# a-r-r-o-w/finetrainers

Measured on NVIDIA H100. Metric: latent_tokens_per_sec, higher is better.
Workload: dtype bf16

## Files before the change

### finetrainers_b200/csrc/b2d_attn.cu

```cuda
#include <float.h>
#include <stdlib.h>
#include <type_traits>
#include "b2d_internal.h"
#include "b2d_ptx.cuh"

namespace b2d {

constexpr int ATT_THREADS = 384;
constexpr int TILE = 128;
constexpr int PANEL = 64;
constexpr int TILE_PANEL_BYTES = TILE * PANEL * 2;
constexpr int HALF_PANEL_BYTES = 64 * PANEL * 2;
constexpr int ATT_SMEM_LIMIT = 227 * 1024;
constexpr float LOG2E = 1.4426950408889634f;
constexpr float LN2 = 0.6931471805599453f;

template <int HD>
struct AttnShape {
    static_assert(HD == 64 || HD == 128, "attention is built for head_dim 64 and 128");
    static constexpr int PANELS = HD / PANEL;
    static constexpr int TILE_BYTES = PANELS * TILE_PANEL_BYTES;
};

__device__ __forceinline__ float fast_exp2(float x) {
    float y;
    asm("ex2.approx.ftz.f32 %0, %1;" : "=f"(y) : "f"(x));
    return y;
}

template <int KK>
__device__ __forceinline__ void acc_to_a(const float (&s)[8 * KK], uint32_t (&a)[KK][4]) {
#pragma unroll
    for (int kk = 0; kk < KK; ++kk) {
        a[kk][0] = pack_bf16x2(s[8 * kk + 0], s[8 * kk + 1]);
        a[kk][1] = pack_bf16x2(s[8 * kk + 2], s[8 * kk + 3]);
        a[kk][2] = pack_bf16x2(s[8 * kk + 4], s[8 * kk + 5]);
        a[kk][3] = pack_bf16x2(s[8 * kk + 6], s[8 * kk + 7]);
    }
}

template <int N, int HD, int XP, int YP>
__device__ __forceinline__ void mma_xyt(float (&s)[N / 2], uint32_t x_smem, uint32_t y_smem) {
    const uint32_t xlo = sdesc_lo_kmajor(x_smem), ylo = sdesc_lo_kmajor(y_smem);
#pragma unroll
    for (int k = 0; k < HD / 16; ++k) {
        const uint32_t xk = xlo + (k / 4) * (XP >> 4) + (k % 4) * SDESC_KSTEP_KMAJOR;
        const uint32_t yk = ylo + (k / 4) * (YP >> 4) + (k % 4) * SDESC_KSTEP_KMAJOR;
        Wgmma<N, 0, 0>::ss(s, sdesc(xk), sdesc(yk), k > 0 ? 1u : 0u);
    }
}

template <int KK, int HD, int ZP>
__device__ __forceinline__ void mma_az(float (&o)[HD / 2], const uint32_t (&a)[KK][4], uint32_t z_smem) {
    const uint32_t zlo = HD == PANEL ? sdesc_lo_mnmajor(z_smem) : sdesc_lo_mnmajor(z_smem, ZP);
#pragma unroll
    for (int kk = 0; kk < KK; ++kk) Wgmma<HD, 0, 1>::rs(o, a[kk], sdesc(zlo + kk * SDESC_KSTEP_MNMAJOR), 1u);
}

template <int HD, int P>
__device__ __forceinline__ void tma_load_tile(uint8_t* dst, const CUtensorMap* m, uint64_t* bar, int h, int row, int b) {
#pragma unroll
    for (int i = 0; i < HD / PANEL; ++i) tma_load_4d(dst + i * P, m, bar, i * PANEL, h, row, b);
}

struct AttnFwdParams {
    CUtensorMap tmQ, tmK, tmV;
    const float* key_bias;
    __nv_bfloat16* out;
    float* lse;
    int B, H, Sq, Sk;
    float scale_log2;
};

template <int HD>
constexpr int FWD_STAGES = HD == 64 ? 3 : 2;
template <int HD>
constexpr int FWD_SMEM = AttnShape<HD>::TILE_BYTES  + FWD_STAGES<HD> * 2 * AttnShape<HD>::TILE_BYTES  + 1024 + 256;
static_assert(FWD_SMEM<64> <= ATT_SMEM_LIMIT && FWD_SMEM<128> <= ATT_SMEM_LIMIT, "attn_fwd shared memory");

template <int HD>
__global__ void __launch_bounds__(ATT_THREADS, 1) attn_fwd_kernel(const __grid_constant__ AttnFwdParams p) {
    constexpr int TILE_BYTES = AttnShape<HD>::TILE_BYTES, STAGES = FWD_STAGES<HD>;
    griddep_launch_dependents();
    extern __shared__ uint8_t smem_raw[];
    uint8_t* smem = reinterpret_cast<uint8_t*>((reinterpret_cast<uintptr_t>(smem_raw) + 1023) & ~uintptr_t(1023));
    uint8_t* sQ = smem;
    uint8_t* sKV = smem + TILE_BYTES;
    uint64_t* q_bar = reinterpret_cast<uint64_t*>(sKV + STAGES * 2 * TILE_BYTES);
    uint64_t* full_bar = q_bar + 1;
    uint64_t* empty_bar = full_bar + STAGES;

    const int warp = threadIdx.x >> 5, lane = threadIdx.x & 31;
    const int qt = blockIdx.x, bh = blockIdx.y;
    const int b = bh / p.H, h = bh % p.H;
    const int n_kt = (p.Sk + TILE - 1) / TILE;

    if (threadIdx.x == 0) {
        tma_prefetch_desc(&p.tmQ);
        tma_prefetch_desc(&p.tmK);
        tma_prefetch_desc(&p.tmV);
        mbar_init(q_bar, 1);
        for (int i = 0; i < STAGES; ++i) {
            mbar_init(&full_bar[i], 1);
            mbar_init(&empty_bar[i], 256);
        }
        fence_mbar_init();
    }
    __syncthreads();
    griddep_wait();

    if (warp < 4) {
        setmaxnreg_dec<40>();
        if (warp == 0 && elect_one()) {
            mbar_expect_tx(q_bar, TILE_BYTES);
            tma_load_tile<HD, TILE_PANEL_BYTES>(sQ, &p.tmQ, q_bar, h, qt * TILE, b);
            int stage = 0;
            uint32_t phase = 0;
            for (int j = 0; j < n_kt; ++j) {
                mbar_wait(&empty_bar[stage], phase ^ 1);
                uint8_t* sK = sKV + stage * 2 * TILE_BYTES;
                mbar_expect_tx(&full_bar[stage], 2 * TILE_BYTES);
                tma_load_tile<HD, TILE_PANEL_BYTES>(sK, &p.tmK, &full_bar[stage], h, j * TILE, b);
                tma_load_tile<HD, TILE_PANEL_BYTES>(sK + TILE_BYTES, &p.tmV, &full_bar[stage], h, j * TILE, b);
                if (++stage == STAGES) {
                    stage = 0;
                    phase ^= 1;
                }
            }
        }
        return;
    }
    setmaxnreg_inc<232>();
    const int cw = (warp >> 2) - 1, wq = warp & 3;
    const int qd = lane & 3;
    const uint32_t q_smem = smem_u32(sQ) + cw * HALF_PANEL_BYTES;
    const float* kb = p.key_bias ? p.key_bias + (long long)b * p.Sk : nullptr;
    const float sl2 = p.scale_log2;

    float kbias[32];
    auto bias_of = [&](int key) { return (kb != nullptr && key < p.Sk) ? kb[key] * LOG2E : 0.f; };
    auto load_bias = [&](int j) {
        if (HD != 64) return;
#pragma unroll
        for (int jj = 0; jj < 16; ++jj)
#pragma unroll
            for (int e = 0; e < 2; ++e) {
                const int key = j * TILE + 8 * jj + 2 * qd + e;
                kbias[2 * jj + e] = bias_of(key);
            }
    };
    float o[HD / 2];
#pragma unroll
    for (int i = 0; i < HD / 2; ++i) o[i] = 0.f;
    float m[2] = {-FLT_MAX, -FLT_MAX}, l[2] = {0.f, 0.f};
    auto softmax = [&](float (&s)[64], int j, float (&corr)[2]) {
        float mx[2] = {-INFINITY, -INFINITY};
        if ((j + 1) * TILE > p.Sk) {
#pragma unroll
            for (int jj = 0; jj < 16; ++jj)
#pragma unroll
                for (int e = 0; e < 2; ++e) {
                    const int key = j * TILE + 8 * jj + 2 * qd + e;
                    const float bias = HD == 64 ? kbias[2 * jj + e] : bias_of(key);
#pragma unroll
                    for (int hh = 0; hh < 2; ++hh) {
                        float v = key < p.Sk ? fmaf(s[4 * jj + 2 * hh + e], sl2, bias) : -INFINITY;
                        s[4 * jj + 2 * hh + e] = v;
                        mx[hh] = fmaxf(mx[hh], v);
                    }
                }
        } else {
#pragma unroll
            for (int jj = 0; jj < 16; ++jj)
#pragma unroll
                for (int e = 0; e < 2; ++e) {
                    const float bias = HD == 64 ? kbias[2 * jj + e] : bias_of(j * TILE + 8 * jj + 2 * qd + e);
#pragma unroll
                    for (int hh = 0; hh < 2; ++hh) {
                        float v = fmaf(s[4 * jj + 2 * hh + e], sl2, bias);
                        s[4 * jj + 2 * hh + e] = v;
                        mx[hh] = fmaxf(mx[hh], v);
                    }
                }
        }
#pragma unroll
        for (int hh = 0; hh < 2; ++hh) {
            mx[hh] = fmaxf(mx[hh], __shfl_xor_sync(0xffffffffu, mx[hh], 1));
            mx[hh] = fmaxf(mx[hh], __shfl_xor_sync(0xffffffffu, mx[hh], 2));
            const float mn = fmaxf(m[hh], mx[hh]);
            corr[hh] = fast_exp2(m[hh] - mn);
            m[hh] = mn;
            l[hh] *= corr[hh];
        }
#pragma unroll
        for (int jj = 0; jj < 16; ++jj)
#pragma unroll
            for (int hh = 0; hh < 2; ++hh)
#pragma unroll
                for (int e = 0; e < 2; ++e) {
                    const float pv = fast_exp2(s[4 * jj + 2 * hh + e] - m[hh]);
                    s[4 * jj + 2 * hh + e] = pv;
                    l[hh] += pv;
                }
    };
    auto rescale_o = [&](const float (&corr)[2]) {
#pragma unroll
        for (int jj = 0; jj < HD / 8; ++jj)
#pragma unroll
            for (int hh = 0; hh < 2; ++hh) {
                o[4 * jj + 2 * hh] *= corr[hh];
                o[4 * jj + 2 * hh + 1] *= corr[hh];
            }
    };
    auto turn_begin = [&] { named_bar_sync(1 + cw, 256); };
    auto turn_end = [&](bool last) {
        if (cw == 0 || !last) named_bar_arrive(2 - cw, 256);
    };
    if (cw == 1) named_bar_arrive(1, 256);

    mbar_wait(q_bar, 0);
    float s[64], corr[2];
    uint32_t pa[8][4];
    int stage = 0;
    uint32_t phase = 0;
    mbar_wait(&full_bar[0], 0);
    turn_begin();
    wgmma_fence();
    mma_xyt<128, HD, TILE_PANEL_BYTES, TILE_PANEL_BYTES>(s, q_smem, smem_u32(sKV));
    wgmma_commit();
    turn_end(false);
    load_bias(0);
    wgmma_wait<0>();
    wgmma_fence_regs(s);
    softmax(s, 0, corr);
    acc_to_a<8>(s, pa);
    for (int j = 1; j < n_kt; ++j) {
        const int prev = stage;
        if (++stage == STAGES) {
            stage = 0;
            phase ^= 1;
        }
        mbar_wait(&full_bar[stage], phase);
        turn_begin();
        wgmma_fence();
        mma_xyt<128, HD, TILE_PANEL_BYTES, TILE_PANEL_BYTES>(s, q_smem, smem_u32(sKV + stage * 2 * TILE_BYTES));
        wgmma_commit();
        mma_az<8, HD, TILE_PANEL_BYTES>(o, pa, smem_u32(sKV + prev * 2 * TILE_BYTES) + TILE_BYTES);
        wgmma_commit();
        turn_end(false);
        load_bias(j);
        wgmma_wait<1>();
        wgmma_fence_regs(s);
        softmax(s, j, corr);
        wgmma_wait<0>();
        wgmma_fence_regs(o);
        mbar_arrive(&empty_bar[prev]);
        rescale_o(corr);
        acc_to_a<8>(s, pa);
    }
    turn_begin();
    wgmma_fence();
    mma_az<8, HD, TILE_PANEL_BYTES>(o, pa, smem_u32(sKV + stage * 2 * TILE_BYTES) + TILE_BYTES);
    wgmma_commit();
    turn_end(true);
    wgmma_wait<0>();
    wgmma_fence_regs(o);
    mbar_arrive(&empty_bar[stage]);
#pragma unroll
    for (int hh = 0; hh < 2; ++hh) {
        l[hh] += __shfl_xor_sync(0xffffffffu, l[hh], 1);
        l[hh] += __shfl_xor_sync(0xffffffffu, l[hh], 2);
    }
    const int r0 = qt * TILE + cw * 64 + wq * 16 + (lane >> 2);
#pragma unroll
    for (int hh = 0; hh < 2; ++hh) {
        const int row = r0 + 8 * hh;
        if (row >= p.Sq) continue;
        const bool any = l[hh] > 0.f;
        const float inv = any ? 1.f / l[hh] : 0.f;
        __nv_bfloat16* orow = p.out + (((long long)b * p.Sq + row) * p.H + h) * HD;
#pragma unroll
        for (int jj = 0; jj < HD / 8; ++jj)
            *reinterpret_cast<uint32_t*>(orow + 8 * jj + 2 * qd) =
                pack_bf16x2(o[4 * jj + 2 * hh] * inv, o[4 * jj + 2 * hh + 1] * inv);
        if (qd == 0) p.lse[(long long)bh * p.Sq + row] = any ? (m[hh] + __log2f(l[hh])) * LN2 : INFINITY;
    }
}

template <int HD>
__global__ void attn_delta_kernel(const __nv_bfloat16* __restrict__ out, const __nv_bfloat16* __restrict__ dout,
                                  const float* __restrict__ lse, float* __restrict__ delta, float* __restrict__ nlse2,
                                  int B, int H, int Sq) {
    constexpr int LANES = HD / 8, LOG2_LANES = HD == 64 ? 3 : 4;
    static_assert((1 << LOG2_LANES) == LANES, "lanes per head row");
    griddep_launch_dependents();
    griddep_wait();
    const long long t = (long long)blockIdx.x * blockDim.x + threadIdx.x;
    const long long total = (long long)B * Sq * H * LANES;
    const bool ok = t < total;
    const long long e0 = (ok ? t : 0) * 8;
    uint4 a = *reinterpret_cast<const uint4*>(out + e0);
    uint4 d = *reinterpret_cast<const uint4*>(dout + e0);
    float acc = bf16_lo(a.x) * bf16_lo(d.x) + bf16_hi(a.x) * bf16_hi(d.x) + bf16_lo(a.y) * bf16_lo(d.y) +
                bf16_hi(a.y) * bf16_hi(d.y) + bf16_lo(a.z) * bf16_lo(d.z) + bf16_hi(a.z) * bf16_hi(d.z) +
                bf16_lo(a.w) * bf16_lo(d.w) + bf16_hi(a.w) * bf16_hi(d.w);
#pragma unroll
    for (int o = 1; o < LANES; o <<= 1) acc += __shfl_xor_sync(0xffffffffu, acc, o);
    if (ok && (t & (LANES - 1)) == 0) {
        const long long hr = t >> LOG2_LANES;
        const int h = (int)(hr % H);
        const long long bq = hr / H;
        const int q = (int)(bq % Sq);
        const int b = (int)(bq / Sq);
        const long long o = ((long long)b * H + h) * Sq + q;
        delta[o] = acc;
        nlse2[o] = -lse[o] * LOG2E;
    }
}

struct AttnBwdParams {
    CUtensorMap tmX1, tmX2, tmY1, tmY2;
    const float* key_bias;
    const float* delta;
    const float* nlse2;
    __nv_bfloat16* out1;
    __nv_bfloat16* out2;
    float* acc1;
    float* acc2;
    long long part_stride;
    int y_per_split;
    int B, H, Sq, Sk;
    float scale, scale_log2;
};

constexpr int ATT_MAX_SPLITS = 8;
template <int HD, int YR>
struct BwdShape {
    static_assert(YR == 64 || YR == 128, "streamed tiles are 64 or 128 rows");
    static constexpr int Y_PANEL_BYTES = YR * PANEL * 2;
    static constexpr int Y_BYTES = AttnShape<HD>::PANELS * Y_PANEL_BYTES;
    static constexpr int COLS = 2 * YR;
    static constexpr int STAGES = HD == 64 && YR == 128 ? 3 : 4;
    static constexpr int SMEM = 2 * AttnShape<HD>::TILE_BYTES + STAGES * (2 * Y_BYTES + COLS * 4) + 1024 + 256;
};
static_assert(BwdShape<64, 64>::SMEM <= ATT_SMEM_LIMIT && BwdShape<64, 128>::SMEM <= ATT_SMEM_LIMIT &&
                  BwdShape<128, 64>::SMEM <= ATT_SMEM_LIMIT,
              "attn_bwd shared memory");
template <int HD>
constexpr int BWD_REGS_PRODUCER = HD == 64 ? 40 : 24;
template <int HD>
constexpr int BWD_REGS_MATH = HD == 64 ? 232 : 240;
static_assert(BWD_REGS_PRODUCER<64> * 128 + BWD_REGS_MATH<64> * 256 == 168 * ATT_THREADS &&
                  BWD_REGS_PRODUCER<128> * 128 + BWD_REGS_MATH<128> * 256 == 168 * ATT_THREADS,
              "setmaxnreg split");

template <bool DKV, int HD, int YR>
__global__ void __launch_bounds__(ATT_THREADS, 1) attn_bwd_kernel(const __grid_constant__ AttnBwdParams p) {
    using Shape = BwdShape<HD, YR>;
    constexpr int TILE_BYTES = AttnShape<HD>::TILE_BYTES, Y_BYTES = Shape::Y_BYTES, STAGES = Shape::STAGES;
    constexpr int COLS = Shape::COLS, KK = YR / 16;
    griddep_launch_dependents();
    extern __shared__ uint8_t smem_raw[];
    uint8_t* smem = reinterpret_cast<uint8_t*>((reinterpret_cast<uintptr_t>(smem_raw) + 1023) & ~uintptr_t(1023));
    uint8_t* sX = smem;
    uint8_t* sY = smem + 2 * TILE_BYTES;
    float* sC = reinterpret_cast<float*>(sY + STAGES * 2 * Y_BYTES);
    uint64_t* x_bar = reinterpret_cast<uint64_t*>(sC + STAGES * COLS);
    uint64_t* full_bar = x_bar + 1;
    uint64_t* empty_bar = full_bar + STAGES;

    const int warp = threadIdx.x >> 5, lane = threadIdx.x & 31;
    const int xt = blockIdx.x, bh = blockIdx.y;
    const int b = bh / p.H, h = bh % p.H;
    const int S_x = DKV ? p.Sk : p.Sq, S_y = DKV ? p.Sq : p.Sk;
    const int y_begin = blockIdx.z * p.y_per_split;
    auto y_end_of_slice = [&] { return min((S_y + YR - 1) / YR, y_begin + p.y_per_split); };

    if (threadIdx.x == 0) {
        tma_prefetch_desc(&p.tmX1);
        tma_prefetch_desc(&p.tmX2);
        tma_prefetch_desc(&p.tmY1);
        tma_prefetch_desc(&p.tmY2);
        mbar_init(x_bar, 1);
        for (int i = 0; i < STAGES; ++i) {
            mbar_init(&full_bar[i], 2);
            mbar_init(&empty_bar[i], 256);
        }
        fence_mbar_init();
    }
    __syncthreads();
    griddep_wait();

    if (warp < 4) {
        setmaxnreg_dec<BWD_REGS_PRODUCER<HD>>();
        const int y_end = y_end_of_slice();
        if (warp == 0 && elect_one()) {
            mbar_expect_tx(x_bar, 2 * TILE_BYTES);
            tma_load_tile<HD, TILE_PANEL_BYTES>(sX, &p.tmX1, x_bar, h, xt * TILE, b);
            tma_load_tile<HD, TILE_PANEL_BYTES>(sX + TILE_BYTES, &p.tmX2, x_bar, h, xt * TILE, b);
            int stage = 0;
            uint32_t phase = 0;
            for (int y = y_begin; y < y_end; ++y) {
                mbar_wait(&empty_bar[stage], phase ^ 1);
                uint8_t* s1 = sY + stage * 2 * Y_BYTES;
                mbar_expect_tx(&full_bar[stage], 2 * Y_BYTES);
                tma_load_tile<HD, Shape::Y_PANEL_BYTES>(s1, &p.tmY1, &full_bar[stage], h, y * YR, b);
                tma_load_tile<HD, Shape::Y_PANEL_BYTES>(s1 + Y_BYTES, &p.tmY2, &full_bar[stage], h, y * YR, b);
                if (++stage == STAGES) {
                    stage = 0;
                    phase ^= 1;
                }
            }
        } else if (warp == 1) {
            const float* kb = p.key_bias ? p.key_bias + (long long)b * p.Sk : nullptr;
            const float* nlse2 = p.nlse2 + (long long)bh * p.Sq;
            const float* delta = p.delta + (long long)bh * p.Sq;
            int stage = 0;
            uint32_t phase = 0;
            for (int y = y_begin; y < y_end; ++y) {
                mbar_wait(&empty_bar[stage], phase ^ 1);
                float* c_off = sC + stage * COLS;
#pragma unroll
                for (int i = lane; i < YR; i += 32) {
                    const int c = y * YR + i;
                    const bool ok = c < S_y;
                    if (DKV) {
                        c_off[i] = ok ? nlse2[c] : 0.f;
                        c_off[YR + i] = ok ? delta[c] : 0.f;
                    } else {
                        c_off[i] = (ok && kb != nullptr) ? kb[c] * LOG2E : 0.f;
                    }
                }
                __syncwarp();
                if (elect_one()) mbar_arrive(&full_bar[stage]);
                if (++stage == STAGES) {
                    stage = 0;
                    phase ^= 1;
                }
            }
// ... 66 lines not shown
    auto y1_of = [&](int st) { return smem_u32(sY + st * 2 * Y_BYTES); };
    auto issue_s_dp = [&] {
        mma_xyt<YR, HD, TILE_PANEL_BYTES, Shape::Y_PANEL_BYTES>(s, x1, y1_of(stage));
        mma_xyt<YR, HD, TILE_PANEL_BYTES, Shape::Y_PANEL_BYTES>(dp, x2, y1_of(stage) + Y_BYTES);
        wgmma_commit();
    };
    auto elementwise_tile = [&](int y) {
        const float* cols = sC + stage * COLS;
        if ((y + 1) * YR > S_y)
            elementwise(y, cols, std::true_type{});
        else
            elementwise(y, cols, std::false_type{});
    };
    uint32_t pa[KK][4], da[KK][4];
    if constexpr (DKV) {
        for (int y = y_begin; y < y_end; ++y) {
            mbar_wait(&full_bar[stage], phase);
            turn_begin();
            wgmma_fence();
            issue_s_dp();
            turn_end(false);
            wgmma_wait<0>();
            wgmma_fence_regs(s);
            wgmma_fence_regs(dp);
            elementwise_tile(y);
            acc_to_a<KK>(dp, da);
            const uint32_t y1 = y1_of(stage);
            turn_begin();
            wgmma_fence();
            acc_to_a<KK>(s, pa);
            mma_az<KK, HD, Shape::Y_PANEL_BYTES>(acc1, pa, y1 + Y_BYTES);
            mma_az<KK, HD, Shape::Y_PANEL_BYTES>(acc2, da, y1);
            wgmma_commit();
            turn_end(y + 1 == y_end);
            wgmma_wait<0>();
            wgmma_fence_regs(acc1);
            wgmma_fence_regs(acc2);
            mbar_arrive(&empty_bar[stage]);
            advance();
        }
    } else {
        mbar_wait(&full_bar[stage], phase);
        turn_begin();
        wgmma_fence();
        issue_s_dp();
        turn_end(false);
        wgmma_wait<0>();
        wgmma_fence_regs(s);
        wgmma_fence_regs(dp);
        elementwise_tile(y_begin);
        acc_to_a<KK>(dp, da);
        for (int y = y_begin + 1; y < y_end; ++y) {
            const int prev = stage;
            advance();
            mbar_wait(&full_bar[stage], phase);
            turn_begin();
            wgmma_fence();
            issue_s_dp();
            mma_az<KK, HD, Shape::Y_PANEL_BYTES>(acc2, da, y1_of(prev));
            wgmma_commit();
            turn_end(false);
            wgmma_wait<1>();
            wgmma_fence_regs(s);
            wgmma_fence_regs(dp);
            elementwise_tile(y);
            wgmma_wait<0>();
            wgmma_fence_regs(acc2);
            mbar_arrive(&empty_bar[prev]);
            acc_to_a<KK>(dp, da);
        }
        turn_begin();
        wgmma_fence();
        mma_az<KK, HD, Shape::Y_PANEL_BYTES>(acc2, da, y1_of(stage));
        wgmma_commit();
        turn_end(true);
        wgmma_wait<0>();
        wgmma_fence_regs(acc2);
        mbar_arrive(&empty_bar[stage]);
    }
#pragma unroll
    for (int hh = 0; hh < 2; ++hh) {
        const int r = r0 + 8 * hh;
        if (r >= S_x) continue;
        const long long base = ((long long)bh * S_x + r) * HD;
#pragma unroll
        for (int jj = 0; jj < HD / 8; ++jj) {
            const int c = 8 * jj + 2 * qd, i = 4 * jj + 2 * hh;
            const float g0 = acc2[i] * p.scale, g1 = acc2[i + 1] * p.scale;
            if (p.acc2 != nullptr) {
                const long long zoff = (long long)blockIdx.z * p.part_stride;
                *reinterpret_cast<float2*>(p.acc2 + zoff + base + c) = make_float2(g0, g1);
                if (DKV) *reinterpret_cast<float2*>(p.acc1 + zoff + base + c) = make_float2(acc1[i], acc1[i + 1]);
            } else {
                *reinterpret_cast<uint32_t*>(p.out2 + base + c) = pack_bf16x2(g0, g1);
                if (DKV) *reinterpret_cast<uint32_t*>(p.out1 + base + c) = pack_bf16x2(acc1[i], acc1[i + 1]);
            }
        }
    }
}

__global__ void attn_dkv_reduce_kernel(const float* __restrict__ part, int splits, long long stride, long long n,
                                       __nv_bfloat16* __restrict__ dv, __nv_bfloat16* __restrict__ dk) {
    griddep_launch_dependents();
    griddep_wait();
    const long long i = ((long long)blockIdx.x * blockDim.x + threadIdx.x) * 4;
    if (i + 3 >= 2 * n) return;
    float4 a = *reinterpret_cast<const float4*>(part + i);
    for (int z = 1; z < splits; ++z) {
        const float4 v = *reinterpret_cast<const float4*>(part + z * stride + i);
        a.x += v.x;
        a.y += v.y;
        a.z += v.z;
        a.w += v.w;
    }
    __nv_bfloat16* dst = i < n ? dv + i : dk + (i - n);
    *reinterpret_cast<uint2*>(dst) = make_uint2(pack_bf16x2(a.x, a.y), pack_bf16x2(a.z, a.w));
}

static int make_head_map(CUtensorMap* m, const void* base, int hd, int B, int H, int S, long long stride_h,
                         long long stride_s, long long stride_b, int box_rows = 128) {
    uint64_t dims[4] = {(uint64_t)hd, (uint64_t)H, (uint64_t)S, (uint64_t)B};
    uint64_t strides[3] = {(uint64_t)stride_h * 2, (uint64_t)stride_s * 2, (uint64_t)stride_b * 2};
    uint32_t box[4] = {PANEL, 1, (uint32_t)box_rows, 1};
    return make_tmap_nd(m, base, 4, dims, strides, box, 2, 1);
}

static int set_smem(const void* kern, int bytes, const char* name) {
    static const void* done_k[64];
    static int done_dev[64];
    static int n_done = 0;
    int dev = 0;
    cudaGetDevice(&dev);
    for (int i = 0; i < n_done; ++i)
        if (done_k[i] == kern && done_dev[i] == dev) return 0;
    cudaError_t e = cudaFuncSetAttribute(kern, cudaFuncAttributeMaxDynamicSharedMemorySize, bytes);
    if (e != cudaSuccess) return set_error(B2D_ERR_CUDA, "cudaFuncSetAttribute(%s): %s", name, cudaGetErrorString(e));
    if (n_done < 64) {
        done_k[n_done] = kern;
        done_dev[n_done] = dev;
        ++n_done;
    }
    return 0;
}

template <int HD>
static int attn_fwd(const void* q, const void* k, const void* v, const float* key_bias, void* out, float* lse, int B,
                    int H, int Sq, int Sk, float scale, cudaStream_t st) {
    AttnFwdParams p;
    memset(&p, 0, sizeof(p));
    int rc;
    if ((rc = make_head_map(&p.tmQ, q, HD, B, H, Sq, (long long)Sq * HD, HD, (long long)H * Sq * HD))) return rc;
    if ((rc = make_head_map(&p.tmK, k, HD, B, H, Sk, (long long)Sk * HD, HD, (long long)H * Sk * HD))) return rc;
    if ((rc = make_head_map(&p.tmV, v, HD, B, H, Sk, (long long)Sk * HD, HD, (long long)H * Sk * HD))) return rc;
    p.key_bias = key_bias;
    p.out = (__nv_bfloat16*)out;
    p.lse = lse;
    p.B = B; p.H = H; p.Sq = Sq; p.Sk = Sk;
    p.scale_log2 = scale * LOG2E;
    if ((rc = set_smem((const void*)attn_fwd_kernel<HD>, FWD_SMEM<HD>, "attn_fwd"))) return rc;
    launch_k(attn_fwd_kernel<HD>, dim3((Sq + TILE - 1) / TILE, B * H), dim3(ATT_THREADS), FWD_SMEM<HD>, st, p);
    B2D_CHECK_LAUNCH("attn_fwd");
    return 0;
}

template <int HD>
static int attn_bwd(const void* q, const void* k, const void* v, const float* key_bias, const void* out,
                    const void* dout, const float* lse, float* delta_ws, void* dq, void* dk, void* dv, int B, int H,
                    int Sq, int Sk, float scale, cudaStream_t st) {
    {
        long long total = (long long)B * Sq * H * (HD / 8);
        launch_k(attn_delta_kernel<HD>, dim3((unsigned)((total + 255) / 256)), dim3(256), 0, st,
                 (const __nv_bfloat16*)out, (const __nv_bfloat16*)dout, lse, delta_ws, delta_ws + (long long)B * H * Sq,
                 B, H, Sq);
        B2D_CHECK_LAUNCH("attn_delta");
    }
    constexpr int YR = HD == 64 ? 128 : 64;
    CUtensorMap mQ, mK, mV, mdO, mQy, mKy, mVy, mdOy;
    int rc;
    const long long hs_q = (long long)Sq * HD, hs_k = (long long)Sk * HD, tok = (long long)H * HD;
    if ((rc = make_head_map(&mQ, q, HD, B, H, Sq, hs_q, HD, H * hs_q))) return rc;
    if ((rc = make_head_map(&mK, k, HD, B, H, Sk, hs_k, HD, H * hs_k))) return rc;
    if ((rc = make_head_map(&mV, v, HD, B, H, Sk, hs_k, HD, H * hs_k))) return rc;
    if ((rc = make_head_map(&mdO, dout, HD, B, H, Sq, HD, tok, Sq * tok))) return rc;
    if ((rc = make_head_map(&mQy, q, HD, B, H, Sq, hs_q, HD, H * hs_q, 64))) return rc;
    if ((rc = make_head_map(&mKy, k, HD, B, H, Sk, hs_k, HD, H * hs_k, 64))) return rc;
    if ((rc = make_head_map(&mVy, v, HD, B, H, Sk, hs_k, HD, H * hs_k, 64))) return rc;
    if ((rc = make_head_map(&mdOy, dout, HD, B, H, Sq, HD, tok, Sq * tok, 64))) return rc;
    const int smem64 = BwdShape<HD, 64>::SMEM, smem_yr = BwdShape<HD, YR>::SMEM;
    if ((rc = set_smem((const void*)attn_bwd_kernel<true, HD, 64>, smem64, "attn_bwd_dkv"))) return rc;
    if ((rc = set_smem((const void*)attn_bwd_kernel<true, HD, YR>, smem_yr, "attn_bwd_dkv"))) return rc;
    if ((rc = set_smem((const void*)attn_bwd_kernel<false, HD, YR>, smem_yr, "attn_bwd_dq"))) return rc;
    AttnBwdParams p;
    memset(&p, 0, sizeof(p));
    p.key_bias = key_bias; p.delta = delta_ws; p.nlse2 = delta_ws + (long long)B * H * Sq;
    p.B = B; p.H = H; p.Sq = Sq; p.Sk = Sk;
    p.scale = scale; p.scale_log2 = scale * LOG2E;
    p.tmX1 = mK; p.tmX2 = mV;
    p.out1 = (__nv_bfloat16*)dv; p.out2 = (__nv_bfloat16*)dk;
    const int n_yq = (Sq + 63) / 64;
    const int kv_ctas = ((Sk + TILE - 1) / TILE) * B * H;
    const int nsm = device_sm_count();
    if (nsm <= 0) return B2D_ERR_CUDA;
    int splits = 1;
    if (Sk <= 512 && kv_ctas < nsm && n_yq >= 8) splits = min(ATT_MAX_SPLITS, min(n_yq / 4, (nsm + kv_ctas - 1) / kv_ctas));
    p.y_per_split = (n_yq + splits - 1) / splits;
    splits = (n_yq + p.y_per_split - 1) / p.y_per_split;
    if (splits > 1) {
        const long long n_kv = (long long)B * H * Sk * HD;
        p.tmY1 = mQy; p.tmY2 = mdOy;
        p.acc1 = delta_ws + 2LL * B * H * Sq;
        p.acc2 = p.acc1 + n_kv;
        p.part_stride = 2 * n_kv;
        launch_k(attn_bwd_kernel<true, HD, 64>, dim3((Sk + TILE - 1) / TILE, B * H, splits), dim3(ATT_THREADS), smem64,
                 st, p);
        B2D_CHECK_LAUNCH("attn_bwd_dkv(split)");
        launch_k(attn_dkv_reduce_kernel, dim3((unsigned)((2 * n_kv / 4 + 255) / 256)), dim3(256), 0, st, (const float*)p.acc1,
                 splits, 2 * n_kv, n_kv, (__nv_bfloat16*)dv, (__nv_bfloat16*)dk);
        B2D_CHECK_LAUNCH("attn_bwd_dkv(reduce)");
    } else {
        p.tmY1 = YR == 128 ? mQ : mQy; p.tmY2 = YR == 128 ? mdO : mdOy;
        p.y_per_split = (Sq + YR - 1) / YR;
        launch_k(attn_bwd_kernel<true, HD, YR>, dim3((Sk + TILE - 1) / TILE, B * H), dim3(ATT_THREADS), smem_yr, st, p);
        B2D_CHECK_LAUNCH("attn_bwd_dkv");
    }
    p.acc1 = p.acc2 = nullptr;
    p.tmX1 = mQ; p.tmX2 = mdO; p.tmY1 = YR == 128 ? mK : mKy; p.tmY2 = YR == 128 ? mV : mVy;
    p.out1 = nullptr; p.out2 = (__nv_bfloat16*)dq;
    p.y_per_split = (Sk + YR - 1) / YR;
    launch_k(attn_bwd_kernel<false, HD, YR>, dim3((Sq + TILE - 1) / TILE, B * H), dim3(ATT_THREADS), smem_yr, st, p);
    B2D_CHECK_LAUNCH("attn_bwd_dq");
    return 0;
}

}

using namespace b2d;

extern "C" int b2d_attn_fwd_hd(const void* q, const void* k, const void* v, const float* key_bias, void* out, float* lse,
                               int32_t B, int32_t H, int32_t Sq, int32_t Sk, int32_t head_dim, float scale,
                               void* stream) {
    B2D_BIND(q);
    if (B <= 0 || H <= 0 || Sq <= 0 || Sk <= 0) return set_error(B2D_ERR_SHAPE, "attn_fwd: bad dims");
    if (head_dim != 64 && head_dim != 128)
        return set_error(B2D_ERR_SHAPE, "attn_fwd: head_dim %d is not supported (64 or 128)", (int)head_dim);
    if (reinterpret_cast<uintptr_t>(out) & 31) return set_error(B2D_ERR_ALIGN, "attn_fwd: out must be 32-byte aligned");
    cudaStream_t st = reinterpret_cast<cudaStream_t>(stream);
    return head_dim == 64 ? b2d::attn_fwd<64>(q, k, v, key_bias, out, lse, B, H, Sq, Sk, scale, st)
                          : b2d::attn_fwd<128>(q, k, v, key_bias, out, lse, B, H, Sq, Sk, scale, st);
}

extern "C" int b2d_attn_bwd_hd(const void* q, const void* k, const void* v, const float* key_bias, const void* out,
                               const void* dout, const float* lse, float* delta_ws, void* dq, void* dk, void* dv,
                               int32_t B, int32_t H, int32_t Sq, int32_t Sk, int32_t head_dim, float scale,
                               void* stream) {
    B2D_BIND(q);
    if (B <= 0 || H <= 0 || Sq <= 0 || Sk <= 0) return set_error(B2D_ERR_SHAPE, "attn_bwd: bad dims");
    if (head_dim != 64 && head_dim != 128)
        return set_error(B2D_ERR_SHAPE, "attn_bwd: head_dim %d is not supported (64 or 128)", (int)head_dim);
    cudaStream_t st = reinterpret_cast<cudaStream_t>(stream);
    return head_dim == 64
               ? b2d::attn_bwd<64>(q, k, v, key_bias, out, dout, lse, delta_ws, dq, dk, dv, B, H, Sq, Sk, scale, st)
               : b2d::attn_bwd<128>(q, k, v, key_bias, out, dout, lse, delta_ws, dq, dk, dv, B, H, Sq, Sk, scale, st);
}

extern "C" int b2d_attn_fwd(const void* q, const void* k, const void* v, const float* key_bias, void* out, float* lse,
                            int32_t B, int32_t H, int32_t Sq, int32_t Sk, float scale, void* stream) {
    return b2d_attn_fwd_hd(q, k, v, key_bias, out, lse, B, H, Sq, Sk, 64, scale, stream);
}

extern "C" int b2d_attn_bwd(const void* q, const void* k, const void* v, const float* key_bias, const void* out,
                            const void* dout, const float* lse, float* delta_ws, void* dq, void* dk, void* dv,
                            int32_t B, int32_t H, int32_t Sq, int32_t Sk, float scale, void* stream) {
    return b2d_attn_bwd_hd(q, k, v, key_bias, out, dout, lse, delta_ws, dq, dk, dv, B, H, Sq, Sk, 64, scale, stream);
}
```

### finetrainers_b200/csrc/b2d_ptx.cuh

```cuda
#pragma once
#include <cuda.h>
#include <cuda_runtime.h>
#include <cuda_bf16.h>
#include <stdint.h>
#include "b2d_wgmma.cuh"

namespace b2d {

__device__ __forceinline__ uint32_t smem_u32(const void* p) { return (uint32_t)__cvta_generic_to_shared(p); }

__device__ __forceinline__ bool elect_one() {
    uint32_t pred = 0;
    asm volatile(
        "{\n\t"
        ".reg .pred P;\n\t"
        "elect.sync _|P, 0xffffffff;\n\t"
        "selp.b32 %0, 1, 0, P;\n\t"
        "}\n"
        : "=r"(pred));
    return pred != 0;
}

__device__ __forceinline__ void mbar_init(uint64_t* bar, uint32_t count) {
    asm volatile("mbarrier.init.shared::cta.b64 [%0], %1;" ::"r"(smem_u32(bar)), "r"(count) : "memory");
}
__device__ __forceinline__ void fence_mbar_init() {
    asm volatile("fence.mbarrier_init.release.cluster;" ::: "memory");
}
__device__ __forceinline__ void mbar_expect_tx(uint64_t* bar, uint32_t bytes) {
    asm volatile("mbarrier.arrive.expect_tx.shared::cta.b64 _, [%0], %1;" ::"r"(smem_u32(bar)), "r"(bytes) : "memory");
}
__device__ __forceinline__ void mbar_arrive(uint64_t* bar) {
    asm volatile("mbarrier.arrive.shared::cta.b64 _, [%0];" ::"r"(smem_u32(bar)) : "memory");
}
__device__ __forceinline__ bool mbar_try_wait(uint64_t* bar, uint32_t parity) {
    uint32_t ok;
    asm volatile(
        "{\n\t"
        ".reg .pred P;\n\t"
        "mbarrier.try_wait.parity.shared::cta.b64 P, [%1], %2, %3;\n\t"
        "selp.b32 %0, 1, 0, P;\n\t"
        "}\n"
        : "=r"(ok)
        : "r"(smem_u32(bar)), "r"(parity), "r"(0x989680u)
        : "memory");
    return ok != 0;
}
__device__ __forceinline__ void mbar_wait(uint64_t* bar, uint32_t parity) {
    while (!mbar_try_wait(bar, parity)) {
    }
}

__device__ __forceinline__ void mbar_wait_spin(uint64_t* bar, uint32_t parity) {
    uint32_t ok = 0;
    do {
        asm volatile(
            "{\n\t"
            ".reg .pred P;\n\t"
            "mbarrier.test_wait.parity.shared::cta.b64 P, [%1], %2;\n\t"
            "selp.b32 %0, 1, 0, P;\n\t"
            "}\n"
            : "=r"(ok)
            : "r"(smem_u32(bar)), "r"(parity)
            : "memory");
    } while (!ok);
}

__device__ __forceinline__ void named_bar_sync(uint32_t id, uint32_t threads) {
    asm volatile("bar.sync %0, %1;" ::"r"(id), "r"(threads) : "memory");
}
__device__ __forceinline__ void named_bar_arrive(uint32_t id, uint32_t threads) {
    asm volatile("bar.arrive %0, %1;" ::"r"(id), "r"(threads) : "memory");
}

__device__ __forceinline__ uint32_t cluster_ctarank() {
    uint32_t r;
    asm volatile("mov.u32 %0, %%cluster_ctarank;" : "=r"(r));
    return r;
}
__device__ __forceinline__ void cluster_sync_all() {
    asm volatile("barrier.cluster.arrive.release;\n\tbarrier.cluster.wait.acquire;" ::: "memory");
}
__device__ __forceinline__ void mbar_arrive_cluster(uint64_t* bar, uint32_t cta) {
    asm volatile(
        "{\n\t"
        ".reg .b32 ra;\n\t"
        "mapa.shared::cluster.u32 ra, %0, %1;\n\t"
        "mbarrier.arrive.shared::cluster.b64 _, [ra];\n\t"
        "}\n" ::"r"(smem_u32(bar)), "r"(cta)
        : "memory");
}

__device__ __forceinline__ void fence_proxy_async_smem() { asm volatile("fence.proxy.async.shared::cta;" ::: "memory"); }

__device__ __forceinline__ void tma_prefetch_desc(const CUtensorMap* m) {
    asm volatile("prefetch.tensormap [%0];" ::"l"(reinterpret_cast<uint64_t>(m)) : "memory");
}
__device__ __forceinline__ void tma_load_2d(void* smem_dst, const CUtensorMap* m, uint64_t* bar, int c0, int c1) {
    asm volatile(
        "cp.async.bulk.tensor.2d.shared::cluster.global.mbarrier::complete_tx::bytes [%0], [%1, {%3, %4}], [%2];"
        ::"r"(smem_u32(smem_dst)), "l"(reinterpret_cast<uint64_t>(m)), "r"(smem_u32(bar)), "r"(c0), "r"(c1)
        : "memory");
}
__device__ __forceinline__ void tma_load_2d_mc(void* smem_dst, const CUtensorMap* m, uint64_t* bar, int c0, int c1,
                                               uint16_t cta_mask) {
    asm volatile(
        "cp.async.bulk.tensor.2d.shared::cluster.global.mbarrier::complete_tx::bytes.multicast::cluster [%0], [%1, {%3, %4}], [%2], %5;"
        ::"r"(smem_u32(smem_dst)), "l"(reinterpret_cast<uint64_t>(m)), "r"(smem_u32(bar)), "r"(c0), "r"(c1), "h"(cta_mask)
        : "memory");
}
__device__ __forceinline__ void tma_load_3d(void* smem_dst, const CUtensorMap* m, uint64_t* bar, int c0, int c1, int c2) {
    asm volatile(
        "cp.async.bulk.tensor.3d.shared::cluster.global.mbarrier::complete_tx::bytes [%0], [%1, {%3, %4, %5}], [%2];"
        ::"r"(smem_u32(smem_dst)), "l"(reinterpret_cast<uint64_t>(m)), "r"(smem_u32(bar)), "r"(c0), "r"(c1), "r"(c2)
        : "memory");
}
__device__ __forceinline__ void tma_load_4d(void* smem_dst, const CUtensorMap* m, uint64_t* bar, int c0, int c1, int c2,
                                            int c3) {
    asm volatile(
        "cp.async.bulk.tensor.4d.shared::cluster.global.mbarrier::complete_tx::bytes [%0], [%1, {%3, %4, %5, %6}], [%2];"
        ::"r"(smem_u32(smem_dst)), "l"(reinterpret_cast<uint64_t>(m)), "r"(smem_u32(bar)), "r"(c0), "r"(c1), "r"(c2),
        "r"(c3)
        : "memory");
}
__device__ __forceinline__ void bulk_load_1d(void* smem_dst, const void* gsrc, uint32_t bytes, uint64_t* bar) {
    asm volatile("cp.async.bulk.shared::cluster.global.mbarrier::complete_tx::bytes [%0], [%1], %2, [%3];" ::"r"(
                     smem_u32(smem_dst)),
                 "l"(gsrc), "r"(bytes), "r"(smem_u32(bar))
                 : "memory");
}
__device__ __forceinline__ void tma_reduce_add_3d(const CUtensorMap* m, const void* smem_src, int c0, int c1, int c2) {
    asm volatile("cp.reduce.async.bulk.tensor.3d.global.shared::cta.add.bulk_group [%0, {%2, %3, %4}], [%1];" ::"l"(
                     reinterpret_cast<uint64_t>(m)),
                 "r"(smem_u32(smem_src)), "r"(c0), "r"(c1), "r"(c2)
                 : "memory");
}
__device__ __forceinline__ void tma_store_3d(const CUtensorMap* m, const void* smem_src, int c0, int c1, int c2) {
    asm volatile("cp.async.bulk.tensor.3d.global.shared::cta.bulk_group [%0, {%2, %3, %4}], [%1];" ::"l"(
                     reinterpret_cast<uint64_t>(m)),
                 "r"(smem_u32(smem_src)), "r"(c0), "r"(c1), "r"(c2)
                 : "memory");
}
__device__ __forceinline__ void tma_store_commit() { asm volatile("cp.async.bulk.commit_group;" ::: "memory"); }
template <int N>
__device__ __forceinline__ void tma_store_wait_read() {
    asm volatile("cp.async.bulk.wait_group.read %0;" ::"n"(N) : "memory");
}
template <int N>
__device__ __forceinline__ void tma_store_wait_all() {
    asm volatile("cp.async.bulk.wait_group %0;" ::"n"(N) : "memory");
}

#ifndef B2D_NO_PDL
__device__ __forceinline__ void griddep_launch_dependents() { asm volatile("griddepcontrol.launch_dependents;" ::: "memory"); }
__device__ __forceinline__ void griddep_wait() { asm volatile("griddepcontrol.wait;" ::: "memory"); }
#else
__device__ __forceinline__ void griddep_launch_dependents() {}
__device__ __forceinline__ void griddep_wait() {}
#endif

__device__ __forceinline__ void sts128(uint32_t addr, uint32_t a, uint32_t b, uint32_t c, uint32_t d) {
    asm volatile("st.shared.v4.b32 [%0], {%1, %2, %3, %4};" ::"r"(addr), "r"(a), "r"(b), "r"(c), "r"(d) : "memory");
}
__device__ __forceinline__ float4 lds128f(uint32_t addr) {
    float4 v;
    asm volatile("ld.shared.v4.f32 {%0, %1, %2, %3}, [%4];" : "=f"(v.x), "=f"(v.y), "=f"(v.z), "=f"(v.w) : "r"(addr));
    return v;
}
__device__ __forceinline__ void sts32(uint32_t addr, uint32_t v) {
    asm volatile("st.shared.b32 [%0], %1;" ::"r"(addr), "r"(v) : "memory");
}
__device__ __forceinline__ uint32_t lds32(uint32_t addr) {
    uint32_t v;
    asm volatile("ld.shared.b32 %0, [%1];" : "=r"(v) : "r"(addr));
    return v;
}
__device__ __forceinline__ uint4 lds128(uint32_t addr) {
    uint4 v;
    asm volatile("ld.shared.v4.b32 {%0, %1, %2, %3}, [%4];" : "=r"(v.x), "=r"(v.y), "=r"(v.z), "=r"(v.w) : "r"(addr));
    return v;
}

constexpr uint32_t SDESC_HI_SW128 = (1024u >> 4) | (1u << 30);
__device__ __forceinline__ uint32_t sdesc_lo_kmajor(uint32_t smem_addr) { return ((smem_addr & 0x3FFFF) >> 4) | (1u << 16); }
__device__ __forceinline__ uint32_t sdesc_lo_mnmajor(uint32_t smem_addr) { return ((smem_addr & 0x3FFFF) >> 4) | (512u << 16); }
__device__ __forceinline__ uint32_t sdesc_lo_mnmajor(uint32_t smem_addr, uint32_t lbo_bytes) {
    return ((smem_addr & 0x3FFFF) >> 4) | ((lbo_bytes >> 4) << 16);
}
constexpr uint32_t SDESC_KSTEP_KMAJOR = 32 >> 4;
constexpr uint32_t SDESC_KSTEP_MNMAJOR = 2048 >> 4;
__device__ __forceinline__ uint64_t sdesc(uint32_t lo) { return ((uint64_t)SDESC_HI_SW128 << 32) | lo; }

template <int R>
__device__ __forceinline__ void setmaxnreg_inc() { asm volatile("setmaxnreg.inc.sync.aligned.u32 %0;" ::"n"(R)); }
template <int R>
__device__ __forceinline__ void setmaxnreg_dec() { asm volatile("setmaxnreg.dec.sync.aligned.u32 %0;" ::"n"(R)); }

__device__ __forceinline__ uint32_t pack_bf16x2(float lo, float hi) {
    __nv_bfloat162 v = __floats2bfloat162_rn(lo, hi);
    return *reinterpret_cast<uint32_t*>(&v);
}
__device__ __forceinline__ float2 unpack_bf16x2(uint32_t u) {
    __nv_bfloat162 v = *reinterpret_cast<__nv_bfloat162*>(&u);
    return __bfloat1622float2(v);
}
__device__ __forceinline__ float bf16_lo(uint32_t u) { return __uint_as_float(u << 16); }
__device__ __forceinline__ float bf16_hi(uint32_t u) { return __uint_as_float(u & 0xffff0000u); }

__device__ __forceinline__ float warp_sum(float v) {
#pragma unroll
    for (int o = 16; o > 0; o >>= 1) v += __shfl_xor_sync(0xffffffffu, v, o);
    return v;
}
__device__ __forceinline__ float warp_max(float v) {
#pragma unroll
    for (int o = 16; o > 0; o >>= 1) v = fmaxf(v, __shfl_xor_sync(0xffffffffu, v, o));
    return v;
}

__device__ __forceinline__ float tanh_approx(float x) {
    float y;
    asm("tanh.approx.f32 %0, %1;" : "=f"(y) : "f"(x));
    return y;
}
__device__ __forceinline__ float gelu_tanh(float x) {
    const float k0 = 0.7978845608028654f, k0k1 = 0.7978845608028654f * 0.044715f;
    float x2 = x * x;
    float t = tanh_approx(x * fmaf(k0k1, x2, k0));
    float hx = 0.5f * x;
    return fmaf(hx, t, hx);
}
__device__ __forceinline__ float dgelu_tanh(float x) {
    const float k0 = 0.7978845608028654f, k0k1 = 0.7978845608028654f * 0.044715f;
    float x2 = x * x;
    float t = tanh_approx(x * fmaf(k0k1, x2, k0));
    float du = fmaf(3.f * k0k1, x2, k0);
    float s = fmaf(-t, t, 1.f);
    return fmaf(0.5f * x * s, du, fmaf(0.5f, t, 0.5f));
}
__device__ __forceinline__ float silu(float x) { return __fdividef(x, 1.f + __expf(-x)); }

}
```

Measured before the change: 39270.

## Make attention forward persistent with double-buffered Q and TMA output stores

Turns the forward attention kernel into a persistent kernel with one CTA per SM that loops over (q-tile, batch, head) work items. Q is double-buffered so the producer can prefetch the next item's Q and K/V while the current one finishes. The output goes through shared memory with a swizzled layout and is written by TMA store instead of per-thread global writes. It also specializes the kernel on whether a key bias is present and uses a tree max reduction for head_dim 64; this adds shared memory use and more complex barrier/phase bookkeeping across items.

```diff
diff --git a/finetrainers_b200/csrc/b2d_attn.cu b/finetrainers_b200/csrc/b2d_attn.cu
--- a/finetrainers_b200/csrc/b2d_attn.cu
+++ b/finetrainers_b200/csrc/b2d_attn.cu
@@ -65,8 +65,8 @@
 
 struct AttnFwdParams {
     CUtensorMap tmQ, tmK, tmV;
+    CUtensorMap tmO;
     const float* key_bias;
-    __nv_bfloat16* out;
     float* lse;
     int B, H, Sq, Sk;
     float scale_log2;
@@ -75,31 +75,35 @@
 template <int HD>
 constexpr int FWD_STAGES = HD == 64 ? 3 : 2;
 template <int HD>
-constexpr int FWD_SMEM = AttnShape<HD>::TILE_BYTES  + FWD_STAGES<HD> * 2 * AttnShape<HD>::TILE_BYTES  + 1024 + 256;
+constexpr int FWD_SMEM = 2 * AttnShape<HD>::TILE_BYTES  + FWD_STAGES<HD> * 2 * AttnShape<HD>::TILE_BYTES  + 1024 + 256;
 static_assert(FWD_SMEM<64> <= ATT_SMEM_LIMIT && FWD_SMEM<128> <= ATT_SMEM_LIMIT, "attn_fwd shared memory");
 
-template <int HD>
+template <int HD, bool BIAS>
 __global__ void __launch_bounds__(ATT_THREADS, 1) attn_fwd_kernel(const __grid_constant__ AttnFwdParams p) {
     constexpr int TILE_BYTES = AttnShape<HD>::TILE_BYTES, STAGES = FWD_STAGES<HD>;
     griddep_launch_dependents();
     extern __shared__ uint8_t smem_raw[];
     uint8_t* smem = reinterpret_cast<uint8_t*>((reinterpret_cast<uintptr_t>(smem_raw) + 1023) & ~uintptr_t(1023));
     uint8_t* sQ = smem;
-    uint8_t* sKV = smem + TILE_BYTES;
-    uint64_t* q_bar = reinterpret_cast<uint64_t*>(sKV + STAGES * 2 * TILE_BYTES);
-    uint64_t* full_bar = q_bar + 1;
+    uint8_t* sKV = smem + 2 * TILE_BYTES;
+    uint64_t* q_full = reinterpret_cast<uint64_t*>(sKV + STAGES * 2 * TILE_BYTES);
+    uint64_t* q_empty = q_full + 2;
+    uint64_t* full_bar = q_empty + 2;
     uint64_t* empty_bar = full_bar + STAGES;
 
     const int warp = threadIdx.x >> 5, lane = threadIdx.x & 31;
-    const int qt = blockIdx.x, bh = blockIdx.y;
-    const int b = bh / p.H, h = bh % p.H;
+    const int n_qt = (p.Sq + TILE - 1) / TILE, n_items = n_qt * p.B * p.H;
     const int n_kt = (p.Sk + TILE - 1) / TILE;
 
     if (threadIdx.x == 0) {
         tma_prefetch_desc(&p.tmQ);
         tma_prefetch_desc(&p.tmK);
         tma_prefetch_desc(&p.tmV);
-        mbar_init(q_bar, 1);
+        tma_prefetch_desc(&p.tmO);
+        for (int i = 0; i < 2; ++i) {
+            mbar_init(&q_full[i], 1);
+            mbar_init(&q_empty[i], 2);
+        }
         for (int i = 0; i < STAGES; ++i) {
             mbar_init(&full_bar[i], 1);
             mbar_init(&empty_bar[i], 256);
@@ -112,19 +116,25 @@
     if (warp < 4) {
         setmaxnreg_dec<40>();
         if (warp == 0 && elect_one()) {
-            mbar_expect_tx(q_bar, TILE_BYTES);
-            tma_load_tile<HD, TILE_PANEL_BYTES>(sQ, &p.tmQ, q_bar, h, qt * TILE, b);
             int stage = 0;
             uint32_t phase = 0;
-            for (int j = 0; j < n_kt; ++j) {
-                mbar_wait(&empty_bar[stage], phase ^ 1);
-                uint8_t* sK = sKV + stage * 2 * TILE_BYTES;
-                mbar_expect_tx(&full_bar[stage], 2 * TILE_BYTES);
-                tma_load_tile<HD, TILE_PANEL_BYTES>(sK, &p.tmK, &full_bar[stage], h, j * TILE, b);
-                tma_load_tile<HD, TILE_PANEL_BYTES>(sK + TILE_BYTES, &p.tmV, &full_bar[stage], h, j * TILE, b);
-                if (++stage == STAGES) {
-                    stage = 0;
-                    phase ^= 1;
+            for (int it = blockIdx.x, n = 0; it < n_items; it += gridDim.x, ++n) {
+                const int qt = it % n_qt, bh = it / n_qt;
+                const int b = bh / p.H, h = bh % p.H;
+                const int qb = n & 1;
+                if (n >= 2) mbar_wait(&q_empty[qb], ((n >> 1) - 1) & 1);
+                mbar_expect_tx(&q_full[qb], TILE_BYTES);
+                tma_load_tile<HD, TILE_PANEL_BYTES>(sQ + qb * TILE_BYTES, &p.tmQ, &q_full[qb], h, qt * TILE, b);
+                for (int j = 0; j < n_kt; ++j) {
+                    mbar_wait(&empty_bar[stage], phase ^ 1);
+                    uint8_t* sK = sKV + stage * 2 * TILE_BYTES;
+                    mbar_expect_tx(&full_bar[stage], 2 * TILE_BYTES);
+                    tma_load_tile<HD, TILE_PANEL_BYTES>(sK, &p.tmK, &full_bar[stage], h, j * TILE, b);
+                    tma_load_tile<HD, TILE_PANEL_BYTES>(sK + TILE_BYTES, &p.tmV, &full_bar[stage], h, j * TILE, b);
+                    if (++stage == STAGES) {
+                        stage = 0;
+                        phase ^= 1;
+                    }
                 }
             }
         }
@@ -133,26 +143,33 @@
     setmaxnreg_inc<232>();
     const int cw = (warp >> 2) - 1, wq = warp & 3;
     const int qd = lane & 3;
-    const uint32_t q_smem = smem_u32(sQ) + cw * HALF_PANEL_BYTES;
-    const float* kb = p.key_bias ? p.key_bias + (long long)b * p.Sk : nullptr;
+    const bool store_thread = (threadIdx.x & 127) == 0;
     const float sl2 = p.scale_log2;
+    const float* kb = nullptr;
 
     float kbias[32];
-    auto bias_of = [&](int key) { return (kb != nullptr && key < p.Sk) ? kb[key] * LOG2E : 0.f; };
+    auto bias_of = [&](int key) { return (BIAS && key < p.Sk) ? kb[key] * LOG2E : 0.f; };
     auto load_bias = [&](int j) {
-        if (HD != 64) return;
-#pragma unroll
-        for (int jj = 0; jj < 16; ++jj)
-#pragma unroll
-            for (int e = 0; e < 2; ++e) {
-                const int key = j * TILE + 8 * jj + 2 * qd + e;
-                kbias[2 * jj + e] = bias_of(key);
-            }
+        if constexpr (HD == 64 && BIAS) {
+#pragma unroll
+            for (int jj = 0; jj < 16; ++jj)
+#pragma unroll
+                for (int e = 0; e < 2; ++e) {
+                    const int key = j * TILE + 8 * jj + 2 * qd + e;
+                    kbias[2 * jj + e] = bias_of(key);
+                }
+        }
+    };
+    auto tile_bias = [&](int key, int i) {
+        if constexpr (!BIAS)
+            return 0.f;
+        else if constexpr (HD == 64)
+            return kbias[i];
+        else
+            return bias_of(key);
     };
     float o[HD / 2];
-#pragma unroll
-    for (int i = 0; i < HD / 2; ++i) o[i] = 0.f;
-    float m[2] = {-FLT_MAX, -FLT_MAX}, l[2] = {0.f, 0.f};
+    float m[2], l[2];
     auto softmax = [&](float (&s)[64], int j, float (&corr)[2]) {
         float mx[2] = {-INFINITY, -INFINITY};
         if ((j + 1) * TILE > p.Sk) {
@@ -161,7 +178,7 @@
 #pragma unroll
                 for (int e = 0; e < 2; ++e) {
                     const int key = j * TILE + 8 * jj + 2 * qd + e;
-                    const float bias = HD == 64 ? kbias[2 * jj + e] : bias_of(key);
+                    const float bias = tile_bias(key, 2 * jj + e);
 #pragma unroll
                     for (int hh = 0; hh < 2; ++hh) {
                         float v = key < p.Sk ? fmaf(s[4 * jj + 2 * hh + e], sl2, bias) : -INFINITY;
@@ -174,14 +191,29 @@
             for (int jj = 0; jj < 16; ++jj)
 #pragma unroll
                 for (int e = 0; e < 2; ++e) {
-                    const float bias = HD == 64 ? kbias[2 * jj + e] : bias_of(j * TILE + 8 * jj + 2 * qd + e);
+                    const float bias = tile_bias(j * TILE + 8 * jj + 2 * qd + e, 2 * jj + e);
 #pragma unroll
                     for (int hh = 0; hh < 2; ++hh) {
                         float v = fmaf(s[4 * jj + 2 * hh + e], sl2, bias);
                         s[4 * jj + 2 * hh + e] = v;
-                        mx[hh] = fmaxf(mx[hh], v);
+                        if (HD != 64) mx[hh] = fmaxf(mx[hh], v);
                     }
                 }
+            if constexpr (HD == 64) {
+#pragma unroll
+                for (int hh = 0; hh < 2; ++hh) {
+                    float t[16];
+#pragma unroll
+                    for (int jj = 0; jj < 16; ++jj) t[jj] = fmaxf(s[4 * jj + 2 * hh], s[4 * jj + 2 * hh + 1]);
+#pragma unroll
+                    for (int i = 0; i < 8; ++i) t[i] = fmaxf(t[i], t[i + 8]);
+#pragma unroll
+                    for (int i = 0; i < 4; ++i) t[i] = fmaxf(t[i], t[i + 4]);
+#pragma unroll
+                    for (int i = 0; i < 2; ++i) t[i] = fmaxf(t[i], t[i + 2]);
+                    mx[hh] = fmaxf(t[0], t[1]);
+                }
+            }
         }
 #pragma unroll
         for (int hh = 0; hh < 2; ++hh) {
@@ -218,73 +250,105 @@
     };
     if (cw == 1) named_bar_arrive(1, 256);
 
-    mbar_wait(q_bar, 0);
     float s[64], corr[2];
     uint32_t pa[8][4];
     int stage = 0;
     uint32_t phase = 0;
-    mbar_wait(&full_bar[0], 0);
-    turn_begin();
-    wgmma_fence();
-    mma_xyt<128, HD, TILE_PANEL_BYTES, TILE_PANEL_BYTES>(s, q_smem, smem_u32(sKV));
-    wgmma_commit();
-    turn_end(false);
-    load_bias(0);
-    wgmma_wait<0>();
-    wgmma_fence_regs(s);
-    softmax(s, 0, corr);
-    acc_to_a<8>(s, pa);
-    for (int j = 1; j < n_kt; ++j) {
-        const int prev = stage;
+    auto advance = [&] {
         if (++stage == STAGES) {
             stage = 0;
             phase ^= 1;
         }
+    };
+    for (int it = blockIdx.x, n = 0; it < n_items; it += gridDim.x, ++n) {
+        const int qt = it % n_qt, bh = it / n_qt;
+        const int b = bh / p.H, h = bh % p.H;
+        const int qb = n & 1;
+        const bool last_item = it + gridDim.x >= n_items;
+        if (BIAS) kb = p.key_bias + (long long)b * p.Sk;
+        uint8_t* sQw = sQ + qb * TILE_BYTES + cw * HALF_PANEL_BYTES;
+        const uint32_t q_smem = smem_u32(sQw);
+#pragma unroll
+        for (int i = 0; i < HD / 2; ++i) o[i] = 0.f;
+#pragma unroll
+        for (int hh = 0; hh < 2; ++hh) {
+            m[hh] = -FLT_MAX;
+            l[hh] = 0.f;
+        }
+        mbar_wait(&q_full[qb], (n >> 1) & 1);
         mbar_wait(&full_bar[stage], phase);
         turn_begin();
         wgmma_fence();
         mma_xyt<128, HD, TILE_PANEL_BYTES, TILE_PANEL_BYTES>(s, q_smem, smem_u32(sKV + stage * 2 * TILE_BYTES));
         wgmma_commit();
-        mma_az<8, HD, TILE_PANEL_BYTES>(o, pa, smem_u32(sKV + prev * 2 * TILE_BYTES) + TILE_BYTES);
+        turn_end(false);
+        if (n > 0 && store_thread) {
+            tma_store_wait_read<0>();
+            mbar_arrive(&q_empty[qb ^ 1]);
+        }
+        load_bias(0);
+        wgmma_wait<0>();
+        wgmma_fence_regs(s);
+        softmax(s, 0, corr);
+        acc_to_a<8>(s, pa);
+        for (int j = 1; j < n_kt; ++j) {
+            const int prev = stage;
+            advance();
+            mbar_wait(&full_bar[stage], phase);
+            turn_begin();
+            wgmma_fence();
+            mma_xyt<128, HD, TILE_PANEL_BYTES, TILE_PANEL_BYTES>(s, q_smem, smem_u32(sKV + stage * 2 * TILE_BYTES));
+            wgmma_commit();
+            mma_az<8, HD, TILE_PANEL_BYTES>(o, pa, smem_u32(sKV + prev * 2 * TILE_BYTES) + TILE_BYTES);
+            wgmma_commit();
+            turn_end(false);
+            load_bias(j);
+            wgmma_wait<1>();
+            wgmma_fence_regs(s);
+            softmax(s, j, corr);
+            wgmma_wait<0>();
+            wgmma_fence_regs(o);
+            mbar_arrive(&empty_bar[prev]);
+            rescale_o(corr);
+            acc_to_a<8>(s, pa);
+        }
+        turn_begin();
+        wgmma_fence();
+        mma_az<8, HD, TILE_PANEL_BYTES>(o, pa, smem_u32(sKV + stage * 2 * TILE_BYTES) + TILE_BYTES);
         wgmma_commit();
-        turn_end(false);
-        load_bias(j);
-        wgmma_wait<1>();
-        wgmma_fence_regs(s);
-        softmax(s, j, corr);
+        turn_end(last_item);
         wgmma_wait<0>();
         wgmma_fence_regs(o);
-        mbar_arrive(&empty_bar[prev]);
-        rescale_o(corr);
-        acc_to_a<8>(s, pa);
-    }
-    turn_begin();
-    wgmma_fence();
-    mma_az<8, HD, TILE_PANEL_BYTES>(o, pa, smem_u32(sKV + stage * 2 * TILE_BYTES) + TILE_BYTES);
-    wgmma_commit();
-    turn_end(true);
-    wgmma_wait<0>();
-    wgmma_fence_regs(o);
-    mbar_arrive(&empty_bar[stage]);
-#pragma unroll
-    for (int hh = 0; hh < 2; ++hh) {
-        l[hh] += __shfl_xor_sync(0xffffffffu, l[hh], 1);
-        l[hh] += __shfl_xor_sync(0xffffffffu, l[hh], 2);
-    }
-    const int r0 = qt * TILE + cw * 64 + wq * 16 + (lane >> 2);
-#pragma unroll
-    for (int hh = 0; hh < 2; ++hh) {
-        const int row = r0 + 8 * hh;
-        if (row >= p.Sq) continue;
-        const bool any = l[hh] > 0.f;
-        const float inv = any ? 1.f / l[hh] : 0.f;
-        __nv_bfloat16* orow = p.out + (((long long)b * p.Sq + row) * p.H + h) * HD;
-#pragma unroll
-        for (int jj = 0; jj < HD / 8; ++jj)
-            *reinterpret_cast<uint32_t*>(orow + 8 * jj + 2 * qd) =
-                pack_bf16x2(o[4 * jj + 2 * hh] * inv, o[4 * jj + 2 * hh + 1] * inv);
-        if (qd == 0) p.lse[(long long)bh * p.Sq + row] = any ? (m[hh] + __log2f(l[hh])) * LN2 : INFINITY;
-    }
+        mbar_arrive(&empty_bar[stage]);
+        advance();
+#pragma unroll
+        for (int hh = 0; hh < 2; ++hh) {
+            l[hh] += __shfl_xor_sync(0xffffffffu, l[hh], 1);
+            l[hh] += __shfl_xor_sync(0xffffffffu, l[hh], 2);
+        }
+        const int r0 = qt * TILE + cw * 64 + wq * 16 + (lane >> 2);
+#pragma unroll
+        for (int hh = 0; hh < 2; ++hh) {
+            const int row = r0 + 8 * hh, r = wq * 16 + (lane >> 2) + 8 * hh;
+            const bool any = l[hh] > 0.f;
+            const float inv = any ? 1.f / l[hh] : 0.f;
+#pragma unroll
+            for (int jj = 0; jj < HD / 8; ++jj)
+                sts32(q_smem + (jj / 8) * TILE_PANEL_BYTES + r * 128 + (((jj % 8) ^ (r & 7)) << 4) + 4 * qd,
+                      pack_bf16x2(o[4 * jj + 2 * hh] * inv, o[4 * jj + 2 * hh + 1] * inv));
+            if (qd == 0 && row < p.Sq) p.lse[(long long)bh * p.Sq + row] = any ? (m[hh] + __log2f(l[hh])) * LN2 : INFINITY;
+        }
+        fence_proxy_async_smem();
+        named_bar_sync(3 + cw, 128);
+        if (store_thread) {
+            if (qt * TILE + cw * 64 < p.Sq)
+#pragma unroll
+                for (int i = 0; i < HD / PANEL; ++i)
+                    tma_store_4d(&p.tmO, sQw + i * TILE_PANEL_BYTES, i * PANEL, h, qt * TILE + cw * 64, b);
+            tma_store_commit();
+        }
+    }
+    if (store_thread) tma_store_wait_all<0>();
 }
 
 template <int HD>
@@ -657,13 +721,17 @@
     if ((rc = make_head_map(&p.tmQ, q, HD, B, H, Sq, (long long)Sq * HD, HD, (long long)H * Sq * HD))) return rc;
     if ((rc = make_head_map(&p.tmK, k, HD, B, H, Sk, (long long)Sk * HD, HD, (long long)H * Sk * HD))) return rc;
     if ((rc = make_head_map(&p.tmV, v, HD, B, H, Sk, (long long)Sk * HD, HD, (long long)H * Sk * HD))) return rc;
+    if ((rc = make_head_map(&p.tmO, out, HD, B, H, Sq, HD, (long long)H * HD, (long long)Sq * H * HD, 64))) return rc;
     p.key_bias = key_bias;
-    p.out = (__nv_bfloat16*)out;
     p.lse = lse;
     p.B = B; p.H = H; p.Sq = Sq; p.Sk = Sk;
     p.scale_log2 = scale * LOG2E;
-    if ((rc = set_smem((const void*)attn_fwd_kernel<HD>, FWD_SMEM<HD>, "attn_fwd"))) return rc;
-    launch_k(attn_fwd_kernel<HD>, dim3((Sq + TILE - 1) / TILE, B * H), dim3(ATT_THREADS), FWD_SMEM<HD>, st, p);
+    const int nsm = device_sm_count();
+    if (nsm <= 0) return B2D_ERR_CUDA;
+    const int items = ((Sq + TILE - 1) / TILE) * B * H;
+    auto kern = key_bias ? attn_fwd_kernel<HD, true> : attn_fwd_kernel<HD, false>;
+    if ((rc = set_smem((const void*)kern, FWD_SMEM<HD>, "attn_fwd"))) return rc;
+    launch_k(kern, dim3(min(items, nsm)), dim3(ATT_THREADS), FWD_SMEM<HD>, st, p);
     B2D_CHECK_LAUNCH("attn_fwd");
     return 0;
 }
diff --git a/finetrainers_b200/csrc/b2d_ptx.cuh b/finetrainers_b200/csrc/b2d_ptx.cuh
--- a/finetrainers_b200/csrc/b2d_ptx.cuh
+++ b/finetrainers_b200/csrc/b2d_ptx.cuh
@@ -141,6 +141,12 @@
                  "r"(smem_u32(smem_src)), "r"(c0), "r"(c1), "r"(c2)
                  : "memory");
 }
+__device__ __forceinline__ void tma_store_4d(const CUtensorMap* m, const void* smem_src, int c0, int c1, int c2, int c3) {
+    asm volatile("cp.async.bulk.tensor.4d.global.shared::cta.bulk_group [%0, {%2, %3, %4, %5}], [%1];" ::"l"(
+                     reinterpret_cast<uint64_t>(m)),
+                 "r"(smem_u32(smem_src)), "r"(c0), "r"(c1), "r"(c2), "r"(c3)
+                 : "memory");
+}
 __device__ __forceinline__ void tma_store_commit() { asm volatile("cp.async.bulk.commit_group;" ::: "memory"); }
 template <int N>
 __device__ __forceinline__ void tma_store_wait_read() {
```

Measured after the change: 39750, median of 6. +1.2%, better.
